# nghorbani/moshpp

Hardware: AMD Instinct MI355X
Metric: solved mocap frames/sec (Stage-II) (higher is better)
Workload: dtype f64

## Files before the change

### moshpp_amd/csrc/chain_solve.hip

```cpp
#include "moshii_dev.h"
#include <utility>
#include <type_traits>
#if defined(__HIP_DEVICE_COMPILE__)
#define MOSHII_OPAQUE(x) __asm__ __volatile__("" : "+v"(x))
#else
#define MOSHII_OPAQUE(x) do {} while (0)
#endif
__device__ __forceinline__ double uni64(double v) {
#if defined(__HIP_DEVICE_COMPILE__)
    return __hiloint2double(__builtin_amdgcn_readfirstlane(__double2hiint(v)), __builtin_amdgcn_readfirstlane(__double2loint(v)));
#else
    return v;
#endif
}

namespace moshii {

typedef double v2d __attribute__((vector_size(16)));

#ifdef MOSHII_PROFILE
__device__ long long g_prof[64];
#define MOSHII_TRACE_N 8192
__device__ long long g_trace[8][MOSHII_TRACE_N][4];
#define TRACE_STAMP(co, seq, ev) do { if (threadIdx.x == 0 && blockIdx.x < 8u * (co).G && (blockIdx.x & 7u) == 0u && (seq) < MOSHII_TRACE_N) g_trace[(co).rank][(seq)][(ev)] = wall_clock64(); } while (0)
// ... 1535 lines not shown
        if (j - 1 >= jlo) {
            const double dj = readlane_f64(y[KK] * pl[KK], (j - 1) & 63);
#pragma unroll
            for (int k = 0; k <= KK; ++k) y[k] = fma(-l1[k], dj, y[k]);
        }
    }
}
template <int NBLK, int B>
__device__ __forceinline__ bool big_blocks(const AReg<NBLK>& A, double* Lp, double* Sl, const double* g, double* pinv, int n, int NB) {
    int tid = threadIdx.x;
    MOSHII_OPAQUE(tid);
    const int ty = tid >> 4, tx = tid & 15, lane = tid & 63;
    const int wv = __builtin_amdgcn_readfirstlane(tid >> 6);
    constexpr int CVR = NBLK * 16, WS = 17;
    double* Wp = Sl + 66;
    double* Ux = Wp + CVR * WS;
    if (B >= NB) return true;
    if (wv == 0) {
        const bool bad = (16 * B + 16 <= n) ? big_panel_eliminate<NBLK, B, true>(Lp, Sl, pinv, n, lane)
                                             : big_panel_eliminate<NBLK, B, false>(Lp, Sl, pinv, n, lane);
        if (bad && lane == 0) Sl[65] = 1.0;
    } else if (B + 1 < NB && B >= 1) {
        big_update_mfma<NBLK>(Lp, Ux, pinv, n, B + 1, NB, wv - 1, lane);
    }
    __syncthreads();
    PROF_LAP_EXT(14);
    if (Sl[65] != 0.0) return false;
    if constexpr (B + 1 < NBLK) {
        if (B + 1 < NB) {
            double W[NBLK];
            const int q2 = (B + 1) * 16 + tx;
            const double gq = g[min(q2, n - 1)] * ((q2 < n) ? 1.0 : 0.0);
#pragma unroll
            for (int bi = B + 1; bi < NBLK; ++bi) {
                const double v = (bi * 16 + ty == n) ? gq : A.a[bi * (bi + 1) / 2 + B + 1];
                W[bi] = (B >= 1 && bi < NB) ? v - Ux[bi * 256 + tid] : v;
            }
            const double* wk = Wp + q2 * WS;
#pragma unroll
            for (int jj = 0; jj < 16; ++jj) {
                const double ck = wk[jj] * pinv[16 * B + jj];
#pragma unroll
                for (int bi = B + 1; bi < NBLK; ++bi) W[bi] = fma(-Wp[(bi * 16 + ty) * WS + jj], ck, W[bi]);
            }
            __syncthreads();
#pragma unroll
            for (int bi = B + 1; bi < NBLK; ++bi) {
                const int q1 = bi * 16 + ty;
                Wp[q1 * WS + tx] = (q1 > n || q2 > n) ? 0.0 : W[bi];
            }
            __syncthreads();
            PROF_LAP_EXT(13);
        }
        return big_blocks<NBLK, B + 1>(A, Lp, Sl, g, pinv, n, NB);
    }
    return true;
}
template <int NBLK>
__device__ bool ldl_big(const AReg<NBLK>& A, double* Lp, double* Sl, const double* g, double* d, double* pinv, int n) {
    int tid = threadIdx.x;
    MOSHII_OPAQUE(tid);
    const int ty = tid >> 4, tx = tid & 15, lane = tid & 63;
    const int wv = __builtin_amdgcn_readfirstlane(tid >> 6);
    PROF_BEGIN(); PROF_COUNT(22);
    const int trash = (n + 1) * (n + 2) / 2, zero = trash + 1;
    constexpr int CVR = NBLK * 16, WS = 17;
    double* Wp = Sl + 66;
    const int NB = n / 16 + 1;
    if (tid == 0) { Sl[64] = 0.0; Sl[65] = 0.0; }
    if (tid < 8) Lp[zero + tid] = 0.0;
    {
        const double gq = g[min(tx, n - 1)] * ((tx < n) ? 1.0 : 0.0);
#pragma unroll
        for (int bi = 0; bi < NBLK; ++bi) {
            const int q1 = bi * 16 + ty;
            const double v = (q1 == n) ? gq : A.a[bi * (bi + 1) / 2];
            Wp[q1 * WS + tx] = (q1 > n || tx > n) ? 0.0 : v;
        }
    }
    __syncthreads();
    PROF_MARK();
    const bool ok = big_blocks<NBLK, 0>(A, Lp, Sl, g, pinv, n, NB);
    __syncthreads();
    PROF_LAP(9);
    if (!ok) return false;
    constexpr int NY = (CVR + 63) / 64;
    double* sb0 = Sl + 66;
    const int base = n * (n + 1) / 2;
    double y[NY], pl[NY];
#pragma unroll
    for (int k = 0; k < NY; ++k) {
        y[k] = (wv == 0 && lane + 64 * k < n) ? Lp[base + lane + 64 * k] : 0.0;
        pl[k] = pinv[min(lane + 64 * k, max(n - 1, 0))];
    }
    auto stage = [&](int pnl) {
        double* sb = sb0 + (pnl & 1) * 16 * CVR;
        const int jlo = 16 * pnl, t3 = tid - 64;
        for (int i0 = 0; i0 < jlo + 15; i0 += MOSHII_TPB - 64) {
            const int i = i0 + t3;
            double v[16];
#pragma unroll
            for (int r = 0; r < 16; ++r) {
                const int j = jlo + r;
                v[r] = Lp[(i < j && j < n) ? j * (j + 1) / 2 + i : zero];
            }
            if (i < CVR) {
#pragma unroll
                for (int r = 0; r < 16; ++r) sb[r * CVR + i] = v[r];
            }
        }
    };
    const int PN = (n + 15) / 16;
    if (wv != 0) stage(PN - 1);
    __syncthreads();
    for (int pnl = PN - 1; pnl >= 0; --pnl) {
        if (wv != 0) { if (pnl > 0) stage(pnl - 1); }
        else {
            const double* sb = sb0 + (pnl & 1) * 16 * CVR;
            const int jlo = 16 * pnl, jhi = min(jlo + 15, n - 1);
            switch (pnl >> 2) {
                case 0: big_backsub_panel<NY, 0>(sb, CVR, jlo, jhi, lane, y, pl); break;
                case 1: if constexpr (NY > 1) big_backsub_panel<NY, 1>(sb, CVR, jlo, jhi, lane, y, pl); break;
                case 2: if constexpr (NY > 2) big_backsub_panel<NY, 2>(sb, CVR, jlo, jhi, lane, y, pl); break;
                default: if constexpr (NY > 3) big_backsub_panel<NY, 3>(sb, CVR, jlo, jhi, lane, y, pl); break;
            }
        }
        __syncthreads();
    }
    if (wv == 0) {
#pragma unroll
        for (int k = 0; k < NY; ++k) if (lane + 64 * k < n) d[lane + 64 * k] = y[k] * pl[k];
    }
    __syncthreads();
    PROF_LAP(10);
    return true;
}

template <int NBLK> __device__ __noinline__ bool coop_rs_reduce(unsigned seq_);

template <int NBLK, bool XT, bool COOP = false>
__device__ void assemble(const Ctx& cx, const ChainLayout& ly, const ModelDev& md, const AttachDev& at,
                         const PriorDev& pr, const OptsDev& op, const double* pose, const FrameParams& fp,
                         int n, int ncp, int nkf, int nfree_hand, double* qs, AReg<NBLK>& A, const CoopCtx& co = CoopCtx()) {
    const int tid = threadIdx.x;
    const int LDJ = ly.LDJ, Tm = ly.Tm, NW = at.NW, Nvp = at.Nvp, bd = md.body_dof, nhf = md.nhand_full;
    const int nshp = XT ? n - ncp : 0;
    const int XS = NW * 4 + 2, TS = NW + 1;
    PROF_BEGIN(); PROF_COUNT(21);
    JtJAcc<NBLK> acc;
    acc.zero();
    const bool rows_here = !COOP || co.mhi > co.mlo;
    if (rows_here) {
    for (int e = tid; e < 3 * Tm * LDJ; e += MOSHII_TPB) cx.Jrow[e] = 0.0;
    if (tid < md.K) {
        double R[9], Jl[9];
        rodrigues_dev(&cx.fullpose[3 * tid], R, Jl);
#pragma unroll
        for (int c = 0; c < 3; ++c) {
            const double ax = Jl[0 * 3 + c], ay = Jl[1 * 3 + c], az = Jl[2 * 3 + c];
            cx.acol[tid * 9 + c * 3 + 0] = ax;
            cx.acol[tid * 9 + c * 3 + 1] = ay;
            cx.acol[tid * 9 + c * 3 + 2] = az;
#pragma unroll
            for (int d = 0; d < 3; ++d) {
                const double rx = R[0 * 3 + d], ry = R[1 * 3 + d], rz = R[2 * 3 + d];
                cx.B[tid * 28 + c * 9 + 0 * 3 + d] = ay * rz - az * ry;
                cx.B[tid * 28 + c * 9 + 1 * 3 + d] = az * rx - ax * rz;
                cx.B[tid * 28 + c * 9 + 2 * 3 + d] = ax * ry - ay * rx;
            }
        }
    }
    __syncthreads();
    if (tid < 3 * md.K) {
        const int k = tid / 3, c = tid % 3;
        const double ax = cx.acol[k * 9 + c * 3 + 0], ay = cx.acol[k * 9 + c * 3 + 1], az = cx.acol[k * 9 + c * 3 + 2];
        double ox = ax, oy = ay, oz = az;
        if (k > 0) mat3_vec(&cx.Rw[md.parents[k] * 9], ax, ay, az, ox, oy, oz);
        cx.omega[k * 10 + c * 3 + 0] = ox; cx.omega[k * 10 + c * 3 + 1] = oy; cx.omega[k * 10 + c * 3 + 2] = oz;
    }
    }
    if constexpr (XT) {
        if (nshp > 0 && rows_here) {
            const int E = nshp, KE = md.K * E;
            double* dtv = qs;
            double* qv = qs + (size_t)KE * 3;
            for (int lvl = 0; lvl <= md.maxdepth; ++lvl) {
                const auto* const bl = gptr(md.depth) + md.K;
                const int l0 = bl[md.K + lvl], nl = bl[md.K + lvl + 1] - l0;
                for (int ix = tid; ix < nl * E; ix += MOSHII_TPB) {
                    const int jl = ix / E, e = ix - jl * E;
                    const int j = bl[l0 + jl], it = j * E + e;
                    const auto* js = md.JS + (size_t)it * 3;
                    const double jx = js[0], jy = js[1], jz = js[2];
                    double dx = jx, dy = jy, dz = jz;
                    if (j > 0) {
                        const int p = md.parents[j];
                        const auto* jp = md.JS + ((size_t)p * E + e) * 3;
                        const double* dp = dtv + ((size_t)p * E + e) * 3;
                        double ox, oy, oz;
                        mat3_vec(&cx.Rw[p * 9], jx - jp[0], jy - jp[1], jz - jp[2], ox, oy, oz);
                        dx = dp[0] + ox; dy = dp[1] + oy; dz = dp[2] + oz;
                    }
                    dtv[(size_t)it * 3 + 0] = dx; dtv[(size_t)it * 3 + 1] = dy; dtv[(size_t)it * 3 + 2] = dz;
                    double rx, ry, rz;
                    mat3_vec(&cx.Rw[j * 9], jx, jy, jz, rx, ry, rz);
                    qv[(size_t)it * 3 + 0] = dx - rx; qv[(size_t)it * 3 + 1] = dy - ry; qv[(size_t)it * 3 + 2] = dz - rz;
                }
                __syncthreads();
            }
        }
    }
    const int v_lo = COOP ? fp.v0 : 0, v_hi = COOP ? fp.v1 : fp.nobs;
    for (int tile0 = v_lo; tile0 < v_hi; tile0 += Tm) {
        const int cnt = min(Tm, v_hi - tile0);
        const int ntv = 3 * cnt;
        if (tid < ntv) {
            const int m = cx.visidx[tile0 + tid / 3];
            const int av = 3 * m + tid % 3;
            const double px = cx.vposed[av * 3 + 0], py = cx.vposed[av * 3 + 1], pz = cx.vposed[av * 3 + 2];
            double Tr[9];
#pragma unroll
            for (int e = 0; e < 9; ++e) Tr[e] = 0.0;
            auto influence = [&](int s, int j, double w) {
                double ox, oy, oz;
                mat3_vec(&cx.Rw[j * 9], px - cx.Jl[j * 3 + 0], py - cx.Jl[j * 3 + 1], pz - cx.Jl[j * 3 + 2], ox, oy, oz);
                cx.xjs[tid * XS + s * 4 + 0] = ox + cx.tw[j * 3 + 0];
                cx.xjs[tid * XS + s * 4 + 1] = oy + cx.tw[j * 3 + 1];
                cx.xjs[tid * XS + s * 4 + 2] = oz + cx.tw[j * 3 + 2];
                cx.xjs[tid * XS + s * 4 + 3] = w;
                cx.tjs[tid * TS + s] = j;
#pragma unroll
                for (int e = 0; e < 9; ++e) Tr[e] += w * cx.Rw[j * 9 + e];
            };
            if (NW <= 4) {
                int jj[4];
                double wv[4];
#pragma unroll
                for (int s = 0; s < 4; ++s) { jj[s] = gptr(at.wj)[av * NW + min(s, NW - 1)]; wv[s] = gptr(at.ww)[av * NW + min(s, NW - 1)]; }
#pragma unroll
                for (int s = 0; s < 4; ++s) if (s < NW) influence(s, jj[s], wv[s]);
            } else {
                for (int s = 0; s < NW; ++s) influence(s, gptr(at.wj)[av * NW + s], gptr(at.ww)[av * NW + s]);
            }
#pragma unroll
            for (int e = 0; e < 9; ++e) cx.Trot[tid * 10 + e] = Tr[e];
        } else if (tid >= 128 && tid < 128 + cnt) {
            const int ml = tid - 128;
            const int m = cx.visidx[tile0 + ml];
            const double c[3] = {gptr(at.coef)[m * 3 + 0], gptr(at.coef)[m * 3 + 1], gptr(at.coef)[m * 3 + 2]};
            double mk[3], L[27];
            marker_eval(c, &cx.vpos[(3 * m + 0) * 3], &cx.vpos[(3 * m + 1) * 3], &cx.vpos[(3 * m + 2) * 3], mk, L);
#pragma unroll
            for (int sv = 0; sv < 3; ++sv)
#pragma unroll
                for (int row = 0; row < 3; ++row)
#pragma unroll
                    for (int x = 0; x < 3; ++x) cx.Lm[(ml * 3 + sv) * 10 + row * 3 + x] = L[row * 9 + sv * 3 + x];
#pragma unroll
            for (int i = 0; i < 3; ++i) cx.Jrow[(3 * ml + i) * LDJ + n] = cx.res[m * 3 + i];
        }
        __syncthreads();
        PROF_LAP(4);
        const int bj0 = bd / 3;
        for (int it = tid; it < cnt * nkf; it += MOSHII_TPB) {
            const int kfi = it / cnt, ml = it - kfi * cnt;
            const int k = cx.kfree[kfi];
            const int m = cx.visidx[tile0 + ml];
            const unsigned long long mask = cx.anc[k];
            const double tkx = cx.tw[k * 3 + 0], tky = cx.tw[k * 3 + 1], tkz = cx.tw[k * 3 + 2];
            double om[10];
            {
                const double2* o2 = reinterpret_cast<const double2*>(&cx.omega[k * 10]);
#pragma unroll
                for (int q = 0; q < 5; ++q) { const double2 t2 = o2[q]; om[2 * q] = t2.x; om[2 * q + 1] = t2.y; }
            }
            double r[9];
#pragma unroll
            for (int e = 0; e < 9; ++e) r[e] = 0.0;
            double Bk[28];
            {
                const double2* bp2 = reinterpret_cast<const double2*>(&cx.B[k * 28]);
#pragma unroll
                for (int q = 0; q < 14; ++q) { const double2 t2 = bp2[q]; Bk[2 * q] = t2.x; Bk[2 * q + 1] = t2.y; }
            }
#pragma unroll
            for (int sv = 0; sv < 3; ++sv) {
                const int al = 3 * ml + sv;
                double ax = 0.0, ay = 0.0, az = 0.0;
                for (int s2 = 0; s2 < NW; ++s2) {
                    const int j = cx.tjs[al * TS + s2];
                    const double2* xw = reinterpret_cast<const double2*>(&cx.xjs[al * XS + s2 * 4]);
                    const double2 xy = xw[0], zw = xw[1];
                    const double w = ((mask >> j) & 1ull) ? zw.y : 0.0;
                    ax += w * (xy.x - tkx);
                    ay += w * (xy.y - tky);
                    az += w * (zw.x - tkz);
                }
                double col[9];
#pragma unroll
                for (int c = 0; c < 3; ++c) {
                    col[c * 3 + 0] = om[c * 3 + 1] * az - om[c * 3 + 2] * ay;
                    col[c * 3 + 1] = om[c * 3 + 2] * ax - om[c * 3 + 0] * az;
                    col[c * 3 + 2] = om[c * 3 + 0] * ay - om[c * 3 + 1] * ax;
                }
                {
                    const double cs = (k >= 1) ? 1.0 : 0.0;
                    const int kk = max(k, 1);
                    double pv[28];
                    const auto* pp = gptr(reinterpret_cast<const v2d*>(at.Pj)) + (size_t)((kk - 1) * 3 + sv) * 14 * at.M + m;
#pragma unroll
                    for (int q = 0; q < 14; ++q) { const v2d t2 = pp[(size_t)q * at.M]; pv[2 * q] = t2[0]; pv[2 * q + 1] = t2[1]; }
                    double Tr[10];
                    {
                        const double2* t2p = reinterpret_cast<const double2*>(&cx.Trot[al * 10]);
#pragma unroll
                        for (int q = 0; q < 5; ++q) { const double2 t2 = t2p[q]; Tr[2 * q] = t2.x; Tr[2 * q + 1] = t2.y; }
                    }
#pragma unroll
                    for (int c = 0; c < 3; ++c) {
                        const double* Bc = &Bk[c * 9];
                        double pd[3];
#pragma unroll
                        for (int i = 0; i < 3; ++i) {
                            double sacc = 0.0;
#pragma unroll
                            for (int e = 0; e < 9; ++e) sacc += pv[i * 9 + e] * Bc[e];
                            pd[i] = cs * sacc;
                        }
#pragma unroll
                        for (int i = 0; i < 3; ++i) col[c * 3 + i] += Tr[i * 3 + 0] * pd[0] + Tr[i * 3 + 1] * pd[1] + Tr[i * 3 + 2] * pd[2];
                    }
                }
                double Ls[10];
                {
                    const double2* l2 = reinterpret_cast<const double2*>(&cx.Lm[(ml * 3 + sv) * 10]);
#pragma unroll
                    for (int q = 0; q < 5; ++q) { const double2 t2 = l2[q]; Ls[2 * q] = t2.x; Ls[2 * q + 1] = t2.y; }
                }
#pragma unroll
                for (int row = 0; row < 3; ++row)
#pragma unroll
                    for (int c = 0; c < 3; ++c)
                        r[row * 3 + c] += Ls[row * 3 + 0] * col[c * 3 + 0] + Ls[row * 3 + 1] * col[c * 3 + 1] + Ls[row * 3 + 2] * col[c * 3 + 2];
            }
            if (k < bj0) {
#pragma unroll
                for (int c = 0; c < 3; ++c) {
                    const int q = cx.colq[3 * k + c];
                    if (q >= 0) {
                        cx.Jrow[(3 * ml + 0) * LDJ + q] = fp.wt_data * r[0 * 3 + c];
                        cx.Jrow[(3 * ml + 1) * LDJ + q] = fp.wt_data * r[1 * 3 + c];
                        cx.Jrow[(3 * ml + 2) * LDJ + q] = fp.wt_data * r[2 * 3 + c];
                    }
                }
            } else {
                double* jh = &cx.Jh[((size_t)ml * ly.nhj + (k - bj0)) * 9];
#pragma unroll
                for (int e = 0; e < 9; ++e) jh[e] = r[e];
            }
        }
        if constexpr (XT) {
            if (nshp > 0) {
                const double* qv = qs + (size_t)md.K * nshp * 3;
                for (int it = tid; it < cnt * nshp; it += MOSHII_TPB) {
                    const int e = it / cnt, ml = it - e * cnt;
                    const int m = cx.visidx[tile0 + ml];
                    double r0 = 0.0, r1 = 0.0, r2 = 0.0;
#pragma unroll
                    for (int sv = 0; sv < 3; ++sv) {
                        const int al = 3 * ml + sv, av = 3 * m + sv;
                        const auto* sp = gptr(at.Ssh) + (size_t)e * 3 * Nvp + av;
                        const double sx = sp[0], sy = sp[Nvp], sz = sp[2 * Nvp];
                        const double* Tr = &cx.Trot[al * 10];
                        double dx = Tr[0] * sx + Tr[1] * sy + Tr[2] * sz;
                        double dy = Tr[3] * sx + Tr[4] * sy + Tr[5] * sz;
                        double dz = Tr[6] * sx + Tr[7] * sy + Tr[8] * sz;
                        for (int s2 = 0; s2 < NW; ++s2) {
                            const int j = cx.tjs[al * TS + s2];
                            const double w = cx.xjs[al * XS + s2 * 4 + 3];
                            const double* qq = qv + ((size_t)j * nshp + e) * 3;
                            dx += w * qq[0]; dy += w * qq[1]; dz += w * qq[2];
                        }
                        const double* Ls = &cx.Lm[(ml * 3 + sv) * 10];
                        r0 += Ls[0] * dx + Ls[1] * dy + Ls[2] * dz;
                        r1 += Ls[3] * dx + Ls[4] * dy + Ls[5] * dz;
                        r2 += Ls[6] * dx + Ls[7] * dy + Ls[8] * dz;
                    }
                    cx.Jrow[(3 * ml + 0) * LDJ + ncp + e] = fp.wt_data * r0;
                    cx.Jrow[(3 * ml + 1) * LDJ + ncp + e] = fp.wt_data * r1;
                    cx.Jrow[(3 * ml + 2) * LDJ + ncp + e] = fp.wt_data * r2;
                }
            }
        }
        for (int it = tid; it < cnt * 9; it += MOSHII_TPB) {
            const int ml = it / 9, row = (it % 9) / 3, q = it % 3;
            cx.Jrow[(3 * ml + row) * LDJ + q] = (row == q) ? fp.wt_data : 0.0;
        }
        __syncthreads();
        PROF_LAP(5);
        if (nfree_hand > 0) {
            for (int it = tid; it < cnt * nfree_hand; it += MOSHII_TPB) {
                const int ml = it / nfree_hand, q = ncp - nfree_hand + (it - ml * nfree_hand);
                const int i = cx.colpid[q] - bd;
                double r0 = 0.0, r1 = 0.0, r2 = 0.0;
                const int hlo = md.comp_lo[i], hhi = md.comp_hi[i];
                for (int h0 = hlo; h0 < hhi; h0 += 15) {
                    double ccv[15];
#pragma unroll
                    for (int u = 0; u < 15; ++u) ccv[u] = md.comps[i * nhf + min(h0 + u, hhi - 1)] * ((h0 + u < hhi) ? 1.0 : 0.0);
#pragma unroll
                    for (int u = 0; u < 15; ++u) {
                        const int h = min(h0 + u, hhi - 1), hj = h / 3, c = h - 3 * hj;
                        const double cc = ccv[u];
                        const double* jh = &cx.Jh[((size_t)ml * ly.nhj + hj) * 9];
                        r0 += cc * jh[0 * 3 + c]; r1 += cc * jh[1 * 3 + c]; r2 += cc * jh[2 * 3 + c];
                    }
                }
                cx.Jrow[(3 * ml + 0) * LDJ + q] = fp.wt_data * r0;
                cx.Jrow[(3 * ml + 1) * LDJ + q] = fp.wt_data * r1;
                cx.Jrow[(3 * ml + 2) * LDJ + q] = fp.wt_data * r2;
            }
            __syncthreads();
        }
        PROF_LAP(6);
        acc.accumulate(cx.Jrow, ntv, LDJ);
        __syncthreads();
        PROF_LAP(7);
    }
    const int np_ = op.nbody;
    double pblk[COOP ? AReg<NBLK>::NE : 1];
    if constexpr (COOP) {
        constexpr int NT = JtJAcc<NBLK>::NT, NE = AReg<NBLK>::NE, NUA = 2 * NT, NUP = (NE + 2) / 2;
        const int wv = __builtin_amdgcn_readfirstlane(tid >> 6);
        unsigned seq = coop_begin(cx);
        TRACE_STAMP(co, seq, 0);
        double gqp = 0.0;
        auto exchange = [&](auto l2) {
            constexpr bool L2 = decltype(l2)::value;
            const CoopSlot mine = coop_slot16(co, seq, co.rank);
#pragma unroll
            for (int t = 0; t < NT; ++t)
                if (4 * t + wv < NE) {
                    coop_st16<L2>(mine, (2 * t) * MOSHII_TPB + tid, acc.c[t][0], acc.c[t][1]);
                    coop_st16<L2>(mine, (2 * t + 1) * MOSHII_TPB + tid, acc.c[t][2], acc.c[t][3]);
                }
            if (np_ > 0 && co.rank == co.prior_rank) {
                const int kb = (int)cx.scal[S_KBEST];
                const double w2 = fp.wt_pose * fp.wt_pose;
                AReg<NBLK> P;
                P.zero();
                P.add_prior(w2, pr.halfprec + (size_t)kb * np_ * np_, np_, cx.colprior, n);
                double gq = 0.0;
                if (tid < n) {
                    const int pb = cx.colprior[tid];
                    if (pb >= 0) {
                        const auto* Hk = pr.halfprec + (size_t)kb * np_ * np_ + pb;
                        const auto* mu = pr.means + (size_t)kb * np_;
                        double s0 = 0.0, s1 = 0.0;
                        for (int b0 = 0; b0 < np_; b0 += 32) {
                            double h[32];
#pragma unroll
                            for (int k = 0; k < 32; ++k) h[k] = Hk[(size_t)min(b0 + k, np_ - 1) * np_];
#pragma unroll
                            for (int k = 0; k < 32; k += 2) {
                                const int b = b0 + k;
                                s0 = fma(h[k] * ((b < np_) ? 1.0 : 0.0), cx.xb[min(b, np_ - 1)] - mu[min(b, np_ - 1)], s0);
                                s1 = fma(h[k + 1] * ((b + 1 < np_) ? 1.0 : 0.0), cx.xb[min(b + 1, np_ - 1)] - mu[min(b + 1, np_ - 1)], s1);
                            }
                        }
                        gq = -(w2 * (s0 + s1));
                    }
                }
                double pe[2 * NUP];
#pragma unroll
                for (int e = 0; e < 2 * NUP; ++e) pe[e] = (e < NE) ? P.a[e] : ((e == NE) ? gq : 0.0);
#pragma unroll
                for (int u = 0; u < NUP; ++u) coop_st16<L2>(mine, (NUA + u) * MOSHII_TPB + tid, pe[2 * u], pe[2 * u + 1]);
            }
            constexpr bool RS = NT >= 9;
            double own[RS ? 1 : 4 * NT];
            if constexpr (!RS) {
#pragma unroll
                for (int t = 0; t < NT; ++t)
#pragma unroll
                    for (int i = 0; i < 4; ++i) own[4 * t + i] = acc.c[t][i];
                acc.zero();
            }
#pragma unroll
            for (int e = 0; e < NE; ++e) pblk[e] = 0.0;
            if (coop_publish_wait<L2>(co, cx, seq)) {
                constexpr int RB = (48 / (2 * NT) < 1) ? 1 : ((48 / (2 * NT) > 6) ? 6 : 48 / (2 * NT));
                const bool has_prior = np_ > 0;
                const CoopSlot sp = coop_slot16(co, seq, co.prior_rank);
                if constexpr (RS) {
                    if (has_prior) {
                        double pv[2 * NUP];
#pragma unroll
                        for (int u = 0; u < NUP; ++u) coop_ld16<L2>(sp, (NUA + u) * MOSHII_TPB + tid, pv[2 * u], pv[2 * u + 1]);
#pragma unroll
                        for (int e = 0; e < NE; ++e) pblk[e] = pv[e];
                        gqp = pv[NE];
                    }
                    const bool ok2 = coop_rs_reduce<NBLK>(seq);
                    seq += 1;
                    if (ok2) {
                        const int TPR = (NT + co.G - 1) / co.G;
#pragma unroll
                        for (int t = 0; t < NT; ++t)
                            if (4 * t + wv < NE) {
                                const CoopSlot sr = coop_slot16(co, seq, t / TPR);
                                double w0, w1, w2, w3;
                                coop_ld16<L2>(sr, (2 * t) * MOSHII_TPB + tid, w0, w1);
                                coop_ld16<L2>(sr, (2 * t + 1) * MOSHII_TPB + tid, w2, w3);
                                acc.c[t] = v4d{w0, w1, w2, w3};
                            }
                    }
                } else {
                double pv[2 * NUP];
                if (has_prior && NUP + RB * NUA <= 48) {
#pragma unroll
                    for (int u = 0; u < NUP; ++u) coop_ld16<L2>(sp, (NUA + u) * MOSHII_TPB + tid, pv[2 * u], pv[2 * u + 1]);
                }
                for (int r0 = 0; r0 < co.G; r0 += RB) {
                    double v[RB][4 * NT];
#pragma unroll
                    for (int u = 0; u < RB; ++u) {
                        const CoopSlot sr = coop_slot16(co, seq, min(r0 + u, co.G - 1));
#pragma unroll
                        for (int t = 0; t < NT; ++t)
                            if (4 * t + wv < NE) {
                                coop_ld16<L2>(sr, (2 * t) * MOSHII_TPB + tid, v[u][4 * t], v[u][4 * t + 1]);
                                coop_ld16<L2>(sr, (2 * t + 1) * MOSHII_TPB + tid, v[u][4 * t + 2], v[u][4 * t + 3]);
                            }
                    }
#pragma unroll
                    for (int u = 0; u < RB; ++u) {
                        if (r0 + u < co.G) {
                            const bool mine_ = (r0 + u) == co.rank;
#pragma unroll
                            for (int t = 0; t < NT; ++t)
                                if (4 * t + wv < NE) {
#pragma unroll
                                    for (int i = 0; i < 4; ++i) acc.c[t][i] += mine_ ? own[4 * t + i] : v[u][4 * t + i];
                                }
                        }
                    }
                }
                if (has_prior) {
                    if (NUP + RB * NUA > 48) {
#pragma unroll
                        for (int u = 0; u < NUP; ++u) coop_ld16<L2>(sp, (NUA + u) * MOSHII_TPB + tid, pv[2 * u], pv[2 * u + 1]);
                    }
#pragma unroll
                    for (int e = 0; e < NE; ++e) pblk[e] = pv[e];
                    gqp = pv[NE];
                }
                }
            }
        };
        exchange(std::false_type());
        if (tid < n) cx.dgn[tid] = gqp;
        TRACE_STAMP(co, seq, 3);
        coop_end(cx, seq);
        PROF_LAP(32);
    }
    A.take(acc, cx.big);
    {
        const int ty = tid >> 4, tx = tid & 15, bn = n >> 4;
        if (ty == (n & 15)) {
#pragma unroll
            for (int bi = 0; bi < NBLK; ++bi)
#pragma unroll
                for (int bj = 0; bj <= bi; ++bj)
                    if (bi == bn && bj * 16 + tx < n) cx.g[bj * 16 + tx] = -A.a[bi * (bi + 1) / 2 + bj];
        }
        __syncthreads();
    }
    double* dvec = cx.y;
    const int kb = (np_ > 0) ? (int)cx.scal[S_KBEST] : 0;
    for (int q = tid; q < n; q += MOSHII_TPB) {
        double dg = 0.0, gq = 0.0;
        if (XT && q >= ncp) {
            const int e = q - ncp;
            const double sv_ = pose[md.NP + e];
            const double w2 = op.wt_shape * op.wt_shape;
            dg += w2; gq -= w2 * sv_;
            if (fp.has_stay) { const double y2 = op.wt_shape_stay * op.wt_shape_stay; dg += y2; gq -= y2 * (sv_ - cx.shp0[e]); }
        } else if (q >= 3) {
            const int pid = cx.colpid[q];
            if (fp.has_velo) { const double w2 = fp.wt_velo * fp.wt_velo; dg += w2; gq -= w2 * (pose[pid] - cx.vtarget[pid]); }
            const int pb = cx.colprior[q];
            if (COOP) { gq += cx.dgn[q]; }
            else if (pb >= 0) {
                const auto* Hk = pr.halfprec + (size_t)kb * np_ * np_ + pb;
                const auto* mu = pr.means + (size_t)kb * np_;
                double s0 = 0.0, s1 = 0.0;
                for (int b0 = 0; b0 < np_; b0 += 32) {
                    double h[32];
#pragma unroll
                    for (int k = 0; k < 32; ++k) h[k] = Hk[(size_t)min(b0 + k, np_ - 1) * np_];
#pragma unroll
                    for (int k = 0; k < 32; k += 2) {
                        const int b = b0 + k;
                        s0 = fma(h[k] * ((b < np_) ? 1.0 : 0.0), cx.xb[min(b, np_ - 1)] - mu[min(b, np_ - 1)], s0);
                        s1 = fma(h[k + 1] * ((b + 1 < np_) ? 1.0 : 0.0), cx.xb[min(b + 1, np_ - 1)] - mu[min(b + 1, np_ - 1)], s1);
                    }
                }
                gq -= fp.wt_pose * fp.wt_pose * (s0 + s1);
            }
            if (fp.use_fingers) {
                if (op.nfinger > 0 && pid >= op.finger[0] && pid <= op.finger[op.nfinger - 1]) {
                    const double w2 = fp.wt_poseH * fp.wt_poseH; dg += w2; gq -= w2 * pose[pid];
                }
            }
            if constexpr (XT) {
                if (fp.use_face && op.nface > 0 && pid >= op.face[0] && pid <= op.face[op.nface - 1]) {
                    const double w2 = fp.wt_poseF * fp.wt_poseF; dg += w2; gq -= w2 * pose[pid];
                }
            }
            if (op.njangle > 0)
                for (int i = 0; i < op.njangle; ++i)
                    if (op.jangle[i] == pid) {
                        const double e = exp(pose[pid]);
                        const double r = (e * e) * (fp.wt_pose * op.wt_jangle), d = 2.0 * r;
                        dg += d * d; gq -= d * r;
                    }
        }
        dvec[q] = dg;
        cx.g[q] += gq;
    }
    __syncthreads();
    A.add_diag(dvec, n);
    if constexpr (COOP) {
#pragma unroll
        for (int e = 0; e < AReg<NBLK>::NE; ++e) A.a[e] += pblk[e];
    } else {
        if (np_ > 0) A.add_prior(fp.wt_pose * fp.wt_pose, pr.halfprec + (size_t)kb * np_ * np_, np_, cx.colprior, n);
    }
    __syncthreads();
    PROF_LAP(8);
}

__device__ __forceinline__ Ctx make_ctx(double* lds, const ChainLayout& ly) {
    Ctx cx;
    cx.pose = lds + ly.o_pose; cx.trans = lds + ly.o_trans; cx.pose_t = lds + ly.o_pose_t; cx.trans_t = lds + ly.o_trans_t;
    cx.pose_prev = lds + ly.o_pose_prev; cx.vtarget = lds + ly.o_vtarget; cx.fullpose = lds + ly.o_fullpose;
    cx.Jl = lds + ly.o_Jl; cx.feat = lds + ly.o_feat; cx.B = lds + ly.o_B; cx.omega = lds + ly.o_omega; cx.Rw = lds + ly.o_Rw; cx.tw = lds + ly.o_tw;
    cx.Rloc = lds + ly.o_Rloc; cx.acol = lds + ly.o_acol;
    cx.vshp = lds + ly.o_vshp; cx.shp0 = lds + ly.o_shp0;
    cx.vconst = lds + ly.o_vconst; cx.vposed = lds + ly.o_vposed; cx.vpos = lds + ly.o_vpos; cx.msim = lds + ly.o_msim; cx.res = lds + ly.o_res;
    cx.xb = lds + ly.o_xb; cx.ell = lds + ly.o_ell; cx.score = lds + ly.o_score; cx.px0 = lds + ly.o_px0; cx.ps0 = lds + ly.o_ps0;
    cx.g = lds + ly.o_g; cx.dsd = lds + ly.o_dsd; cx.dgn = lds + ly.o_dgn; cx.ddl = lds + ly.o_ddl; cx.y = lds + ly.o_y;
    cx.red = lds + ly.o_red; cx.scal = lds + ly.o_scal;
    cx.anc = reinterpret_cast<unsigned long long*>(lds + ly.o_anc);
    int* ints = reinterpret_cast<int*>(lds + ly.o_ints);
    cx.visidx = ints + ly.i_visidx; cx.colpid = ints + ly.i_colpid; cx.colprior = ints + ly.i_colprior;
    cx.pid2prior = ints + ly.i_pid2prior; cx.jointslot = ints + ly.i_jointslot; cx.kfree = ints + ly.i_kfree;
    cx.colq = ints + ly.i_colq; cx.ksum = ints + ly.i_ksum; cx.kconst = ints + ly.i_kconst;
    cx.big = lds + ly.o_big;
    cx.Jh = cx.big + ly.t_Jh; cx.Jrow = cx.big + ly.t_Jrow; cx.Lm = cx.big + ly.t_Lm; cx.Trot = cx.big + ly.t_Trot;
    cx.xjs = cx.big + ly.t_xjs; cx.rest = cx.big + ly.t_rest;
    cx.tjs = reinterpret_cast<int*>(cx.big + ly.t_tjs);

    return cx;
}

template <class T>
__device__ __forceinline__ T uniform_load(const T* p) {
    static_assert(sizeof(T) % 4 == 0, "word-sized descriptors only");
    T out;
    int* o = reinterpret_cast<int*>(&out);
    const int* q = reinterpret_cast<const int*>(p);
#pragma unroll
    for (int i = 0; i < (int)(sizeof(T) / 4); ++i) o[i] = __builtin_amdgcn_readfirstlane(q[i]);
    return out;
}

struct KArgsMirror { const ChainDev* chains; ModelDev md; PriorDev pr; OptsDev op; ChainLayout ly; int n_chains; };
#if defined(__HIP_DEVICE_COMPILE__) && !defined(MOSHII_NO_KARGS)
typedef const KArgsMirror __attribute__((address_space(4)))* KArgsPtr;
__device__ __forceinline__ KArgsPtr kargs_of(const KernelCtx* kc) {
    const unsigned long long v = kc->kargs;
    return (KArgsPtr)(((unsigned long long)(unsigned)__builtin_amdgcn_readfirstlane((int)(v >> 32)) << 32) | (unsigned)__builtin_amdgcn_readfirstlane((int)v));
}
#define MOSHII_CTX_FROM_KARGS(kc) const KArgsPtr ka_ = kargs_of(kc); const ChainLayout ly = ka_->ly; const ModelDev md = ka_->md; const PriorDev pr = ka_->pr; const OptsDev op = ka_->op;
#else
#define MOSHII_CTX_FROM_KARGS(kc) const ChainLayout ly = uniform_load(&(kc)->ly); const ModelDev md = uniform_load(&(kc)->md); const PriorDev pr = uniform_load(&(kc)->pr); const OptsDev op = uniform_load(&(kc)->op);
#endif

template <int NBLK>
__device__ __noinline__ bool coop_rs_reduce(unsigned seq_) {
    extern __shared__ __attribute__((aligned(16))) double lds[];
    const KernelCtx* kc = reinterpret_cast<const KernelCtx*>(lds);
    const ChainLayout ly = uniform_load(&kc->ly);
    const Ctx cx = make_ctx(lds, ly);
    const CoopCtx co = uniform_load(&kc->co);
// ... 252 lines not shown
                gather(std::false_type());
                coop_end(cx, seq);
            }
            if (tid == 0) rigid_init_serial(cx, fp, visrow, at.M);
            __syncthreads();
            for (int i = tid; i < NPX; i += MOSHII_TPB) cx.pose_t[i] = cx.pose[i];
            if (tid < 3) cx.trans_t[tid] = cx.trans[tid];
            __syncthreads();
            rigid = false;
            continue;
        }
        if (eval_only) break;
        ++n_fev;
        PROF_T(_t1);
        bool improved = false, do_assemble = false;
        double rho = 0.0;
        if (init) {
            sse = uni64(last.total);
            do_assemble = true;
        } else {
            rho = sse - last.total;
            if (rho > 0.0) rho = rho / (2.0 * gd - dAd);
            improved = rho > 0.0;
            at_pose = improved;
            if (improved) {
                for (int i = tid; i < NPX; i += MOSHII_TPB) cx.pose[i] = cx.pose_t[i];
                if (tid < 3) cx.trans[tid] = cx.trans_t[tid];
                __syncthreads();
                if (e3 > 0.0 && (sse - last.total) / sse < e3) done = true;
                else { do_assemble = true; sse = uni64(last.total); }
            }
        }
        PROF_ACC(23, _t1);
        double pp = 0.0, gg = 0.0, gAg = 0.0;
        if (do_assemble) {
            { PROF_T(_ta); A = APass<NBLK, MOSHII_ASM_RET_VEC(NBLK)>::unpack(assemble_fn<NBLK, XT, COOP>(ly.o_pose, n, ncp, nkf, nfree_hand, qs)); PROF_ACC(16, _ta); }
            if constexpr (COOP) { if (cx.scal[S_COOP_FAIL] != 0.0) break; }
            PROF_T(_t2);
            double gm = 0.0;
            for (int q = tid; q < n; q += MOSHII_TPB) {
                const double gq = cx.g[q];
                const double pq = (q < 3) ? cx.trans[q] : cx.pose[cx.colpid[q]];
                gm = fmax(gm, fabs(gq)); pp += pq * pq; gg += gq * gq;
            }
            gAg = A.quad_partial(cx.g, n, tid);
            block_max_sum3(gm, pp, gg, gAg, cx.red);
            gm = uni64(gm); pp = uni64(pp); gg = uni64(gg); gAg = uni64(gAg);
            if (gm < 1e-15) done = true;
            PROF_ACC(24, _t2);
        }
        PROF_T(_t3);
        if (!init) {
            const double pnorm2 = (improved && do_assemble) ? pp : p2;
            if (rho > 0.9) delta = fmax(delta, 2.5 * step);
            else if (rho < 0.05) delta *= 0.25;
            delta = uni64(delta);
            if (delta <= 1e-15 * sqrt(pnorm2)) done = true;
        }
        if (init || improved) {
            if (!init && iteration >= op.maxiter) done = true;
            if (done) break;
            ++iteration;
            const double csd = gg / gAg;
            norm_sd = uni64(fabs(csd) * sqrt(gg));
            for (int q = tid; q < n; q += MOSHII_TPB) cx.dsd[q] = csd * cx.g[q];
            have_gn = false;
            __syncthreads();
        } else if (done) {
            break;
        }
        init = false;
        PROF_ACC(25, _t3);
        PROF_T(_t4);
        if (norm_sd >= delta) {
            const double sc = delta / norm_sd;
            for (int q = tid; q < n; q += MOSHII_TPB) cx.ddl[q] = sc * cx.dsd[q];
        } else {
            if (!have_gn) {
                constexpr bool BIG = XT && NBLK > 8;
                bool solved;
                PROF_T(_ts);
                if constexpr (BIG) solved = ldl_big<NBLK>(A, qs + (size_t)6 * md.K * op.nshape, cx.big, cx.g, cx.dgn, cx.y, n);
                else solved = ldl_solve<NBLK>(A, ly.o_big, ly.o_g, ly.o_dgn, ly.o_y, n);
                PROF_ACC(17, _ts);
                PROF_ACC(26, _t4);
                if (!solved) {
                    fail = 1;
                    for (int q = tid; q < n; q += MOSHII_TPB) cx.dgn[q] = cx.dsd[q];
                    __syncthreads();
                }
                double sg = 0.0;
                dl_dd = 0.0; dl_gs = 0.0; dl_ds = 0.0;
                for (int q = tid; q < n; q += MOSHII_TPB) {
                    const double dg_ = cx.dgn[q], dsq = cx.dsd[q], df = dg_ - dsq;
                    sg += dg_ * dg_; dl_dd += df * df; dl_gs += dg_ * dsq; dl_ds += df * dsq;
                }
                block_sum4(sg, dl_dd, dl_gs, dl_ds, cx.red);
                dl_dd = uni64(dl_dd); dl_gs = uni64(dl_gs); dl_ds = uni64(dl_ds);
                norm_gn = uni64(sqrt(sg));
                have_gn = true;
            }
            if (norm_gn <= delta) {
                for (int q = tid; q < n; q += MOSHII_TPB) cx.ddl[q] = cx.dgn[q];
            } else {
                const double delta_sq = delta * delta;
                const double sqnorm_sd = norm_sd * norm_sd;
                const double pnow = dl_dd * delta_sq + dl_gs * dl_gs - (norm_gn * norm_gn) * sqnorm_sd;
                const double beta = (delta_sq - sqnorm_sd) / (dl_ds + sqrt(pnow));
                for (int q = tid; q < n; q += MOSHII_TPB) cx.ddl[q] = cx.dsd[q] + beta * (cx.dgn[q] - cx.dsd[q]);
            }
        }
        __syncthreads();
        PROF_T(_t5);
        double s2 = 0.0;
        p2 = 0.0; gd = 0.0;
        for (int q = tid; q < n; q += MOSHII_TPB) {
            const double dq = cx.ddl[q];
            const double pq = (q < 3) ? cx.trans[q] : cx.pose[cx.colpid[q]];
            s2 += dq * dq; p2 += pq * pq; gd += cx.g[q] * dq;
        }
        dAd = A.quad_partial(cx.ddl, n, tid);
        block_sum4(s2, p2, gd, dAd, cx.red);
        p2 = uni64(p2); gd = uni64(gd); dAd = uni64(dAd);
        step = uni64(sqrt(s2));
        if (step <= 1e-15 * sqrt(p2)) break;
        for (int i = tid; i < NPX; i += MOSHII_TPB) cx.pose_t[i] = cx.pose[i];
        if (tid < 3) cx.trans_t[tid] = cx.trans[tid] + cx.ddl[tid];
        __syncthreads();
        for (int q = 3 + tid; q < n; q += MOSHII_TPB) cx.pose_t[cx.colpid[q]] += cx.ddl[q];
        __syncthreads();
        PROF_ACC(27, _t5);
    }
    n_iter += iteration;
    carried = last;
    return last;
}


template <int NBLK, int MINW, bool XT, bool COOP = false>
__global__ __launch_bounds__(MOSHII_TPB, MINW) void k_chain_solve(const ChainDev* __restrict__ chains, ModelDev md, PriorDev pr,
                                                             OptsDev op, ChainLayout ly, int n_chains) {
    extern __shared__ __attribute__((aligned(16))) double lds[];
    const int tid = threadIdx.x;
    int chain_id = blockIdx.x;
    CoopCtx co = CoopCtx();
    if constexpr (COOP) {
        const int G = chains[0].coop.G;
        const int q = blockIdx.x >> 3;
        chain_id = 8 * (q / G) + (blockIdx.x & 7);
        if (chain_id >= n_chains) return;
        const ChainDev* c0 = chains + chain_id;
        co.G = G; co.rank = q % G; co.prior_rank = c0->coop.prior_rank;
        co.mlo = c0->coop.mlo[co.rank]; co.mhi = c0->coop.mlo[co.rank + 1];
        co.slot_doubles = c0->coop.slot_doubles; co.slots = c0->coop.slots; co.flags = c0->coop.flags; co.skew = c0->coop.skew;
    }
    const bool lead = !COOP || co.rank == 0;
    const ChainDev* chp = chains + chain_id;
    const AttachDev at = *chp->att;
    const Ctx cx = make_ctx(lds, ly);
    if (tid == 0) {
        KernelCtx* kc = reinterpret_cast<KernelCtx*>(lds);
        kc->ly = ly; kc->md = md; kc->pr = pr; kc->op = op; kc->at = at;
#if defined(__HIP_DEVICE_COMPILE__)
        kc->kargs = (unsigned long long)__builtin_amdgcn_kernarg_segment_ptr();
#if !defined(MOSHII_NO_KARGS)
        {
            const KArgsPtr kk = (KArgsPtr)__builtin_amdgcn_kernarg_segment_ptr();
            if (kk->chains != chains || kk->n_chains != n_chains || kk->ly.total_doubles != ly.total_doubles || kk->md.V != md.V || kk->op.maxiter != op.maxiter)
                __builtin_trap();
        }
#endif
#endif
        if constexpr (COOP) { kc->co = co; cx.scal[S_COOP_SEQ] = 0.0; cx.scal[S_COOP_FAIL] = 0.0; }
    }

    const int NP = md.NP, M = at.M, F = chp->F, skip = chp->skip;
    bool has_prev, first;
    {
        const double* is = chp->init_state;
        const double* ip = chp->init_pose;
        const double* iv = chp->init_prev;
        const double* it = chp->init_trans;
        for (int i = tid; i < NP; i += MOSHII_TPB) {
            cx.pose[i] = is ? is[i] : (ip ? ip[i] : 0.0);
            cx.pose_prev[i] = is ? is[NP + i] : (iv ? iv[i] : 0.0);
            cx.vtarget[i] = 0.0;
            cx.pid2prior[i] = -1;
        }
        if (tid < 3) cx.trans[tid] = is ? is[2 * NP + tid] : (it ? it[tid] : 0.0);
        if constexpr (XT) {
            const double* ish = chp->init_shape;
            for (int e = tid; e < op.nshape; e += MOSHII_TPB) { cx.pose[NP + e] = is ? is[2 * NP + 5 + e] : (ish ? ish[e] : 0.0); cx.shp0[e] = 0.0; }
        }
        has_prev = is ? (is[2 * NP + 3] != 0.0) : (iv != nullptr);
        first = is ? (is[2 * NP + 4] != 0.0) : (chp->first != 0);
    }
    if (tid == 0) cx.scal[S_PRIOR_REF] = 0.0;
    for (int i = tid; i < 8 * pr.npose + 16; i += MOSHII_TPB) cx.ell[i] = 0.0;
    if (tid < md.K) cx.anc[tid] = md.anc[tid];
    for (int i = tid; i < 3 * md.K; i += MOSHII_TPB) cx.Jl[i] = md.J[i];
    __syncthreads();
    for (int b = tid; b < op.nbody; b += MOSHII_TPB) cx.pid2prior[op.body[b]] = b;
    __syncthreads();
    int vc_key = 0, tab_key = 0;
    int rejoin_run = 0;
    int bi_next = 0;
    bool fuse_on = false;
    bool at_pose = false;
    int fwd_set = 0;
    PROF_BEGIN();
#ifdef MOSHII_PROFILE
    const long long _wall0 = wall_clock64();
#endif

    bool tail_cut = false;
    for (int t = 0; t <= F; ++t) {
        PROF_T(_tf);
        if constexpr (!COOP && !XT) {
            if (chp->tail_done != nullptr && chp->tail_can_cut != 0 && t < F && F - t > chp->tail_left) {
                if (tid == 0) cx.scal[S_ABORT] = (double)__hip_atomic_load(chp->tail_done, __ATOMIC_RELAXED, __HIP_MEMORY_SCOPE_AGENT);
                __syncthreads();
                const bool cut = cx.scal[S_ABORT] >= (double)chp->tail_quota;
                __syncthreads();
                if (cut) {
                    auto spoil = [&](double* so, double flag) {
                        for (int i = tid; i < NP; i += MOSHII_TPB) { so[i] = cx.pose[i]; so[NP + i] = cx.pose_prev[i]; }
                        if (tid < 3) so[2 * NP + tid] = cx.trans[tid];
                        if (tid == 3) so[2 * NP + 3] = flag;
                        if (tid == 4) so[2 * NP + 4] = 0.0;
                    };
                    spoil(chp->entry_state, MOSHII_MARK_ENTRY_SPOILED);
                    spoil(chp->final_state, MOSHII_MARK_FINAL_SPOILED);
                    if (tid == 0 && chp->tail_mark != nullptr) *chp->tail_mark = 0x7fffffff;
                    tail_cut = true;
                    break;
                }
            }
        }
        if constexpr (COOP) {
            if (chp->baton != nullptr || chp->nb > 0 || chp->rejoin_tol > 0.0) {
                bool halt = false;
                if (lead) {
                    const int S = 2 * NP + 5;
                    if (rejoin_run >= 2 && t < F) {
                        if (tid == 0 && chp->frames_done) *chp->frames_done = t;
                        halt = true;
                    }
                    if (!halt && bi_next < chp->nb && t == chp->bnd[bi_next] - chp->bnd_off) {
                        double* s1 = chp->run_final + (size_t)bi_next * S;
                        for (int i = tid; i < NP; i += MOSHII_TPB) { s1[i] = cx.pose[i]; s1[NP + i] = cx.pose_prev[i]; }
                        if (tid < 3) s1[2 * NP + tid] = cx.trans[tid];
                        if (tid == 3) s1[2 * NP + 3] = has_prev ? 1.0 : 0.0;
                        if (tid == 4) s1[2 * NP + 4] = first ? 1.0 : 0.0;
                        if (chp->baton != nullptr) {
                            if (tid == 0) {
                                int* st = chp->baton + 2 * (chp->chunk0 + 1 + bi_next);
                                double go = 1.0;
                                if (__hip_atomic_load(st, __ATOMIC_ACQUIRE, __HIP_MEMORY_SCOPE_AGENT) == 1) {
                                    __hip_atomic_store(st + 1, 1, __ATOMIC_RELEASE, __HIP_MEMORY_SCOPE_AGENT);
                                    int spins = 0;
                                    while (__hip_atomic_load(st, __ATOMIC_ACQUIRE, __HIP_MEMORY_SCOPE_AGENT) != 2) {
                                        __builtin_amdgcn_s_sleep(64);
                                        if (++spins > 20000) { go = 0.0; break; }
                                    }
                                }
                                __builtin_amdgcn_fence(__ATOMIC_ACQUIRE, "agent");
                                cx.scal[S_BATON] = go;
                            }
                            __syncthreads();
                            if (cx.scal[S_BATON] == 0.0) { if (tid == 0 && chp->frames_done) *chp->frames_done = t; halt = true; }
                            __syncthreads();
                        }
                        if (!halt) {
                            double* s2 = chp->run_entry + (size_t)(bi_next + 1) * S;
                            for (int i = tid; i < NP; i += MOSHII_TPB) { s2[i] = cx.pose[i]; s2[NP + i] = cx.pose_prev[i]; }
                            if (tid < 3) s2[2 * NP + tid] = cx.trans[tid];
                            if (tid == 3) s2[2 * NP + 3] = has_prev ? 1.0 : 0.0;
                            if (tid == 4) s2[2 * NP + 4] = first ? 1.0 : 0.0;
                            ++bi_next;
                        }
                    }
                    if (!halt && chp->baton != nullptr && t < F) {
                        if (tid == 0) cx.scal[S_ABORT] = (double)__hip_atomic_load(&chp->baton[2 * chp->chunk0 + 1], __ATOMIC_RELAXED, __HIP_MEMORY_SCOPE_AGENT);
                        __syncthreads();
                        if (cx.scal[S_ABORT] != 0.0) {
                            if (tid == 0) {
                                chp->run_entry[(size_t)bi_next * S + 2 * NP + 3] = MOSHII_MARK_ENTRY_SPOILED;
                                int* mark = chp->abort_at + chp->chunk0 + bi_next;
                                if (*mark < chp->bnd_off + t) *mark = chp->bnd_off + t;
                                if (chp->frames_done) *chp->frames_done = -t - 1;
                            }
                            halt = true;
                        }
                        __syncthreads();
                    }
                }
                const unsigned seq = coop_begin(cx);
                const double mine[1] = {halt ? 1.0 : 0.0};
                const bool okx = coop_exchange_small<1>(co, cx, seq, mine, cx.y);
                const double verdict = okx ? cx.y[0] : 1.0;
                coop_end(cx, seq);
                if (verdict != 0.0) break;
            }
        }
        for (int which = 0; which < 2; ++which) {
            double* so = (which == 0) ? ((t == skip) ? chp->entry_state : nullptr) : ((t == F) ? chp->final_state : nullptr);
// ... 450 lines not shown
```

### moshpp_amd/csrc/moshii_dev.h

```cpp
#pragma once
#include <hip/hip_runtime.h>
#include <stdint.h>
#include "solve_plan.h"

#define MOSHII_MAXK 64

#ifndef MOSHII_AS_GLOBAL
#define MOSHII_AS_GLOBAL __attribute__((address_space(1)))
#endif
template <class T> __device__ __forceinline__ const T MOSHII_AS_GLOBAL* gptr(const T* p) { return (const T MOSHII_AS_GLOBAL*)p; }
template <class T> __device__ __forceinline__ T MOSHII_AS_GLOBAL* gptr(T* p) { return (T MOSHII_AS_GLOBAL*)p; }
#if defined(__HIP_DEVICE_COMPILE__)
template <class T> __device__ __forceinline__ const T MOSHII_AS_GLOBAL* gptr(const T MOSHII_AS_GLOBAL* p) { return p; }
#endif
#if defined(__HIP_DEVICE_COMPILE__)
#define MOSHII_GP(T) T MOSHII_AS_GLOBAL*
#else
#define MOSHII_GP(T) T*
#endif
template <class T> __host__ __device__ inline MOSHII_GP(const T) as_gp(const T* p) { return (MOSHII_GP(const T))p; }
template <class T> __host__ __device__ inline MOSHII_GP(T) as_gp_rw(T* p) { return (MOSHII_GP(T))p; }
#define MOSHII_TPB 256

struct ModelDev {
    int V, K, P, NP, body_dof, hand_dof, nhand_full, maxdepth;
    MOSHII_GP(const int) parents;
    MOSHII_GP(const double) J;
    MOSHII_GP(const double) hands_mean;
    MOSHII_GP(const double) comps;
    MOSHII_GP(const int) comp_lo;
    MOSHII_GP(const int) comp_hi;
    MOSHII_GP(const int) col_lo;
    MOSHII_GP(const int) col_hi;
    MOSHII_GP(const unsigned long long) anc;
    MOSHII_GP(const int) depth;
    int nshape;
    MOSHII_GP(const double) JS;
};

struct AttachDev {
    int M, Nv, Nvp, NW;
    MOSHII_GP(const double) vsh;
    MOSHII_GP(const double) Pt;
    MOSHII_GP(const double) Pj;
    MOSHII_GP(const int) wj;
    MOSHII_GP(const double) ww;
    MOSHII_GP(const double) coef;
    MOSHII_GP(const double) Ssh;
};

struct PriorDev {
    int G, npose;
    MOSHII_GP(const double) means;
    MOSHII_GP(const double) chols;
    MOSHII_GP(const double) halfprec;
    MOSHII_GP(const double) neglogw;
    MOSHII_GP(const double) cnorm;
};

struct OptsDev {
    double wt_data, wt_velo, wt_poseB, wt_poseH, wt_annealing, num_train_markers;
    double e3_first, e3, delta0;
    int maxiter, n1, n2, nbody, nfinger, same_sets;
    MOSHII_GP(const int) step1;
    MOSHII_GP(const int) step2;
    MOSHII_GP(const int) body;
    MOSHII_GP(const int) finger;
    double wt_poseF, wt_shape, wt_shape_stay;
    int nface, nshape;
    MOSHII_GP(const int) face;
    int njangle;
    double wt_jangle;
    MOSHII_GP(const int) jangle;
};

#define MOSHII_COOP_MAXG 8
struct CoopDev {
    int G;
    int prior_rank;
    int mlo[MOSHII_COOP_MAXG + 1];
    int slot_doubles;
    int qstride;
    int skew;
    MOSHII_GP(unsigned long long) slots;
    MOSHII_GP(unsigned int) flags;
};
struct CoopCtx {
    int G, rank, prior_rank, mlo, mhi, slot_doubles, skew;
    MOSHII_GP(unsigned long long) slots;
    MOSHII_GP(unsigned int) flags;
};

struct ChainDev {
    const AttachDev* att;
    int F, first;
    const double* obs;
    const uint8_t* vis;
    const double* init_pose;
    const double* init_trans;
    const double* init_prev;
    double* pose;
    double* fullpose;
    double* trans;
    double* msim;
    double* errs;
    int* iters;
    int* status;
    int skip;
    const double* init_state;
    double* entry_state;
    double* final_state;
    int nb;
    const int* bnd;
    double* run_final;
    double* run_entry;
    int* frames_done;
    int* baton;
    int* abort_at;
    int chunk0;
    int bnd_off;
    const double* init_shape;
    double* shape;
    double* qscratch;
    double rejoin_tol;
    int fuse_F;
    int fuse_c;
    int fuse_has_next;
    int fuse_has_prev;
    int* fuse_flags;
    int* fuse_count;
    double fuse_tol;
    CoopDev coop;
    int* tail_done;
    int tail_quota, tail_left;
    int tail_can_cut;
    int* tail_mark;
};

struct ChainLayout {
    int Mmax, Nvmax, NWmax, nmax, Tm, nkfmax, LDJ, nhj;
    int NPX;
    int o_vshp, o_shp0;
    int o_pose, o_trans, o_pose_t, o_trans_t, o_pose_prev, o_vtarget, o_fullpose;
    int o_feat, o_B, o_omega, o_Rw, o_tw, o_Rloc, o_acol, o_Jl;
    int o_vposed, o_vpos, o_msim, o_res, o_vconst;
    int o_xb, o_ell, o_score;
    int o_px0, o_ps0;
    int o_g, o_dsd, o_dgn, o_ddl, o_y;
    int o_red, o_scal;
    int o_anc;
    int o_ints;
    int o_big;
    int big_doubles;
    int total_doubles;
    int i_visidx, i_colpid, i_colprior, i_pid2prior, i_jointslot, i_kfree, i_colq, i_ksum, i_kconst, i_total;
    int t_Jh, t_Jrow, t_Lm, t_Trot, t_xjs, t_rest, t_tjs;
};

struct KernelCtx {
    ChainLayout ly;
    ModelDev md;
    PriorDev pr;
    OptsDev op;
    AttachDev at;
    double fp_raw[12];
    CoopCtx co;
    unsigned long long kargs;
};
#define MOSHII_KC_DOUBLES ((int)((sizeof(KernelCtx) + 15) / 16 * 2))

struct Lbs32Model {
    float* v_shaped;
    float* posedirs_t;
    float* weights;
    float* J;
    float* hcompf;
    float* hmeanf;
    float* jtab;
    float* hcj;
    int jtab_valid;
    int* varflag;
    int epoch;
    int Vp;
    _Float16* Pfrag;
    int* perm;
    char* tables;
    unsigned tab_gnr;
    unsigned tab_gjid;
    unsigned tab_gx;
    unsigned tab_vshs;
    unsigned tab_vsc;
    unsigned tab_gw;
    long long* dbgbuf;
    int K, NRM;
    float pscale, inv_pscale;
    int NVT, KS;
    int KJ;
    int mfma_ok;
    float* Atr;
    _Float16* featF;
    int Fcap;
    _Float16* PfragX;
    float* JSf;
    float* Sft;
    int nshape, KSX;
    float sxscale;
    long long featcap;
};
```

Before: 65170.

## Overlap joint-axis setup with tile prep and skip empty prior-rank exchange

Wavefront 0 now computes the Rodrigues, B and omega terms by itself, synchronised only with a wave barrier. The vertex-tile threads shift to ids 64 and up, so that setup work runs alongside the first tile's influence computation and one block-wide barrier goes away. The residual copy into Jrow moves after the tile barrier. In the cooperative exchange, a prior-only rank that owns no marker rows no longer posts its accumulator, and readers skip loading its slot and their own slot. This cuts global-memory traffic in the cross-block reduction, but it adds tighter lane-count assumptions, such as K≤64 for the omega loop spread and 3*cnt fitting in threads 64 to 191.

```diff
diff --git a/moshpp_amd/csrc/chain_solve.hip b/moshpp_amd/csrc/chain_solve.hip
--- a/moshpp_amd/csrc/chain_solve.hip
+++ b/moshpp_amd/csrc/chain_solve.hip
@@ -1711,6 +1711,7 @@
     const bool rows_here = !COOP || co.mhi > co.mlo;
     if (rows_here) {
     for (int e = tid; e < 3 * Tm * LDJ; e += MOSHII_TPB) cx.Jrow[e] = 0.0;
+    if (tid < 64) {
     if (tid < md.K) {
         double R[9], Jl[9];
         rodrigues_dev(&cx.fullpose[3 * tid], R, Jl);
@@ -1729,13 +1730,15 @@
             }
         }
     }
-    __syncthreads();
-    if (tid < 3 * md.K) {
-        const int k = tid / 3, c = tid % 3;
+    __builtin_amdgcn_fence(__ATOMIC_ACQ_REL, "wavefront");
+    __builtin_amdgcn_wave_barrier();
+    for (int i = tid; i < 3 * md.K; i += 64) {
+        const int k = i / 3, c = i % 3;
         const double ax = cx.acol[k * 9 + c * 3 + 0], ay = cx.acol[k * 9 + c * 3 + 1], az = cx.acol[k * 9 + c * 3 + 2];
         double ox = ax, oy = ay, oz = az;
         if (k > 0) mat3_vec(&cx.Rw[md.parents[k] * 9], ax, ay, az, ox, oy, oz);
         cx.omega[k * 10 + c * 3 + 0] = ox; cx.omega[k * 10 + c * 3 + 1] = oy; cx.omega[k * 10 + c * 3 + 2] = oz;
+    }
     }
     }
     if constexpr (XT) {
@@ -1770,12 +1773,14 @@
         }
     }
     const int v_lo = COOP ? fp.v0 : 0, v_hi = COOP ? fp.v1 : fp.nobs;
+    if (v_hi <= v_lo) __syncthreads();
     for (int tile0 = v_lo; tile0 < v_hi; tile0 += Tm) {
         const int cnt = min(Tm, v_hi - tile0);
         const int ntv = 3 * cnt;
-        if (tid < ntv) {
-            const int m = cx.visidx[tile0 + tid / 3];
-            const int av = 3 * m + tid % 3;
+        const int tl = tid - 64;
+        if (tl >= 0 && tl < ntv) {
+            const int m = cx.visidx[tile0 + tl / 3];
+            const int av = 3 * m + tl % 3;
             const double px = cx.vposed[av * 3 + 0], py = cx.vposed[av * 3 + 1], pz = cx.vposed[av * 3 + 2];
             double Tr[9];
 #pragma unroll
@@ -1783,11 +1788,11 @@
             auto influence = [&](int s, int j, double w) {
                 double ox, oy, oz;
                 mat3_vec(&cx.Rw[j * 9], px - cx.Jl[j * 3 + 0], py - cx.Jl[j * 3 + 1], pz - cx.Jl[j * 3 + 2], ox, oy, oz);
-                cx.xjs[tid * XS + s * 4 + 0] = ox + cx.tw[j * 3 + 0];
-                cx.xjs[tid * XS + s * 4 + 1] = oy + cx.tw[j * 3 + 1];
-                cx.xjs[tid * XS + s * 4 + 2] = oz + cx.tw[j * 3 + 2];
-                cx.xjs[tid * XS + s * 4 + 3] = w;
-                cx.tjs[tid * TS + s] = j;
+                cx.xjs[tl * XS + s * 4 + 0] = ox + cx.tw[j * 3 + 0];
+                cx.xjs[tl * XS + s * 4 + 1] = oy + cx.tw[j * 3 + 1];
+                cx.xjs[tl * XS + s * 4 + 2] = oz + cx.tw[j * 3 + 2];
+                cx.xjs[tl * XS + s * 4 + 3] = w;
+                cx.tjs[tl * TS + s] = j;
 #pragma unroll
                 for (int e = 0; e < 9; ++e) Tr[e] += w * cx.Rw[j * 9 + e];
             };
@@ -1802,9 +1807,9 @@
                 for (int s = 0; s < NW; ++s) influence(s, gptr(at.wj)[av * NW + s], gptr(at.ww)[av * NW + s]);
             }
 #pragma unroll
-            for (int e = 0; e < 9; ++e) cx.Trot[tid * 10 + e] = Tr[e];
-        } else if (tid >= 128 && tid < 128 + cnt) {
-            const int ml = tid - 128;
+            for (int e = 0; e < 9; ++e) cx.Trot[tl * 10 + e] = Tr[e];
+        } else if (tid >= 192 && tid < 192 + cnt) {
+            const int ml = tid - 192;
             const int m = cx.visidx[tile0 + ml];
             const double c[3] = {gptr(at.coef)[m * 3 + 0], gptr(at.coef)[m * 3 + 1], gptr(at.coef)[m * 3 + 2]};
             double mk[3], L[27];
@@ -1815,11 +1820,15 @@
                 for (int row = 0; row < 3; ++row)
 #pragma unroll
                     for (int x = 0; x < 3; ++x) cx.Lm[(ml * 3 + sv) * 10 + row * 3 + x] = L[row * 9 + sv * 3 + x];
-#pragma unroll
-            for (int i = 0; i < 3; ++i) cx.Jrow[(3 * ml + i) * LDJ + n] = cx.res[m * 3 + i];
         }
         __syncthreads();
         PROF_LAP(4);
+        if (tid >= 192 && tid < 192 + cnt) {
+            const int ml = tid - 192;
+            const int m = cx.visidx[tile0 + ml];
+#pragma unroll
+            for (int i = 0; i < 3; ++i) cx.Jrow[(3 * ml + i) * LDJ + n] = cx.res[m * 3 + i];
+        }
         const int bj0 = bd / 3;
         for (int it = tid; it < cnt * nkf; it += MOSHII_TPB) {
             const int kfi = it / cnt, ml = it - kfi * cnt;
@@ -1997,9 +2006,12 @@
         auto exchange = [&](auto l2) {
             constexpr bool L2 = decltype(l2)::value;
             const CoopSlot mine = coop_slot16(co, seq, co.rank);
+            constexpr bool RS = NT >= 9;
+            const bool bare_prior = !RS && co.prior_bare != 0;
+            const bool post_acc = !(bare_prior && co.rank == co.prior_rank);
 #pragma unroll
             for (int t = 0; t < NT; ++t)
-                if (4 * t + wv < NE) {
+                if (post_acc && 4 * t + wv < NE) {
                     coop_st16<L2>(mine, (2 * t) * MOSHII_TPB + tid, acc.c[t][0], acc.c[t][1]);
                     coop_st16<L2>(mine, (2 * t + 1) * MOSHII_TPB + tid, acc.c[t][2], acc.c[t][3]);
                 }
@@ -2036,7 +2048,6 @@
 #pragma unroll
                 for (int u = 0; u < NUP; ++u) coop_st16<L2>(mine, (NUA + u) * MOSHII_TPB + tid, pe[2 * u], pe[2 * u + 1]);
             }
-            constexpr bool RS = NT >= 9;
             double own[RS ? 1 : 4 * NT];
             if constexpr (!RS) {
 #pragma unroll
@@ -2082,25 +2093,34 @@
                 }
                 for (int r0 = 0; r0 < co.G; r0 += RB) {
                     double v[RB][4 * NT];
+                    auto wanted = [&](int r) { return r < co.G && r != co.rank && !(bare_prior && r == co.prior_rank); };
 #pragma unroll
                     for (int u = 0; u < RB; ++u) {
-                        const CoopSlot sr = coop_slot16(co, seq, min(r0 + u, co.G - 1));
-#pragma unroll
-                        for (int t = 0; t < NT; ++t)
-                            if (4 * t + wv < NE) {
-                                coop_ld16<L2>(sr, (2 * t) * MOSHII_TPB + tid, v[u][4 * t], v[u][4 * t + 1]);
-                                coop_ld16<L2>(sr, (2 * t + 1) * MOSHII_TPB + tid, v[u][4 * t + 2], v[u][4 * t + 3]);
-                            }
-                    }
-#pragma unroll
-                    for (int u = 0; u < RB; ++u) {
-                        if (r0 + u < co.G) {
-                            const bool mine_ = (r0 + u) == co.rank;
+                        if (wanted(r0 + u)) {
+                            const CoopSlot sr = coop_slot16(co, seq, r0 + u);
 #pragma unroll
                             for (int t = 0; t < NT; ++t)
                                 if (4 * t + wv < NE) {
-#pragma unroll
-                                    for (int i = 0; i < 4; ++i) acc.c[t][i] += mine_ ? own[4 * t + i] : v[u][4 * t + i];
+                                    coop_ld16<L2>(sr, (2 * t) * MOSHII_TPB + tid, v[u][4 * t], v[u][4 * t + 1]);
+                                    coop_ld16<L2>(sr, (2 * t + 1) * MOSHII_TPB + tid, v[u][4 * t + 2], v[u][4 * t + 3]);
+                                }
+                        }
+                    }
+#pragma unroll
+                    for (int u = 0; u < RB; ++u) {
+                        if ((r0 + u) == co.rank) {
+#pragma unroll
+                            for (int t = 0; t < NT; ++t)
+                                if (4 * t + wv < NE) {
+#pragma unroll
+                                    for (int i = 0; i < 4; ++i) acc.c[t][i] += own[4 * t + i];
+                                }
+                        } else if (wanted(r0 + u)) {
+#pragma unroll
+                            for (int t = 0; t < NT; ++t)
+                                if (4 * t + wv < NE) {
+#pragma unroll
+                                    for (int i = 0; i < 4; ++i) acc.c[t][i] += v[u][4 * t + i];
                                 }
                         }
                     }
@@ -2659,6 +2679,7 @@
         const ChainDev* c0 = chains + chain_id;
         co.G = G; co.rank = q % G; co.prior_rank = c0->coop.prior_rank;
         co.mlo = c0->coop.mlo[co.rank]; co.mhi = c0->coop.mlo[co.rank + 1];
+        co.prior_bare = c0->coop.mlo[co.prior_rank + 1] == c0->coop.mlo[co.prior_rank];
         co.slot_doubles = c0->coop.slot_doubles; co.slots = c0->coop.slots; co.flags = c0->coop.flags; co.skew = c0->coop.skew;
     }
     const bool lead = !COOP || co.rank == 0;
diff --git a/moshpp_amd/csrc/moshii_dev.h b/moshpp_amd/csrc/moshii_dev.h
--- a/moshpp_amd/csrc/moshii_dev.h
+++ b/moshpp_amd/csrc/moshii_dev.h
@@ -87,6 +87,7 @@
 };
 struct CoopCtx {
     int G, rank, prior_rank, mlo, mhi, slot_doubles, skew;
+    int prior_bare;
     MOSHII_GP(unsigned long long) slots;
     MOSHII_GP(unsigned int) flags;
 };
```

New measurement: 66450, median of 6. +2.0%, better.
